# ArshvirSk/Multimodal-Rare-Disease

Hardware: NVIDIA B200
Metric: fused fwd samples/sec (224² img+128 tok) @1/2/4/8 B200; % tensor-pipe peak (higher is better)
Workload: dtype bf16

## Files before the change

multimodal-rare-disease_b200/csrc/gemm_conv.cu:

```cuda

#include "gemm_conv.h"

#include <stdio.h>
#include <stdlib.h>
#include <string.h>

#include "ptx.cuh"
#include "tma_host.h"

namespace mrd {

namespace {

bool g_use_pdl = true;

int g_debug_ring = -1;
void apply_debug_env() {
    static bool done = false;
    if (done) return;
    done = true;
    if (const char* e = getenv("MRD_DEBUG_PDL")) g_use_pdl = atoi(e) != 0;
    if (const char* e = getenv("MRD_DEBUG_RING")) g_debug_ring = atoi(e);
}

constexpr int kBlockM = 128;
constexpr int kNumThreads = 352;
constexpr int kEpiThreads = 256;
constexpr int kStageBufBytes = 128 * 128;
constexpr int kSmemLimit = 232448;
constexpr int kMaxStages = 8;
constexpr int kMaxRing = 8;
constexpr int kBarBytes = 1024;

constexpr int MODE_GENERIC = 0, MODE_STEM = 1, MODE_FLAT3 = 2;

template <int BLOCK_N, int MODE>
struct Cfg {
    static constexpr bool STEM = MODE == MODE_STEM;
    static constexpr int BLOCK_K = STEM ? 32 : 64;
    static constexpr int ROW_BYTES = BLOCK_K * 2;
    static constexpr int A_STAGE = kBlockM * ROW_BYTES;
    static constexpr int B_STAGE = BLOCK_N * ROW_BYTES;
    static constexpr int STAGE = A_STAGE + B_STAGE;
    static constexpr int FIXED = 2 * kStageBufBytes + kBarBytes + 1024;
    static constexpr int TMEM_COLS = 2 * BLOCK_N;
    static constexpr uint32_t LAYOUT = STEM ? 4u : 2u;
    static constexpr uint32_t SBO = 8 * ROW_BYTES;
};

struct TileCoord {
    int n_idx, w0, h0, n0;
};

__device__ __forceinline__ TileCoord decode_tile(const ConvGemmParams& p, int tile) {
    TileCoord t;
    int m_idx = tile / p.n_tiles_n;
    t.n_idx = tile - m_idx * p.n_tiles_n;
    int tw_i = m_idx % p.tiles_w;
    int r = m_idx / p.tiles_w;
    int th_i = r % p.tiles_h;
    int img_i = r / p.tiles_h;
    t.w0 = tw_i * p.tw + p.w_shift;
    t.h0 = th_i * p.th;
    t.n0 = img_i * p.nb;
    return t;
}

constexpr int kStemRow = 192;
constexpr int kStemRows = 37;

constexpr int kLnStripeBytes = 128 * 8 * 8 + 64;

template <int BLOCK_N, int MODE, bool SPLITK = false, bool EPI2 = false, bool LNC = false, bool PAIR = false>
__global__ void __launch_bounds__(kNumThreads, 1)
conv_gemm_kernel(const __grid_constant__ ConvGemmParams p) {
    using C = Cfg<BLOCK_N, MODE>;
    constexpr bool STEM = MODE == MODE_STEM;
    constexpr bool FLAT = MODE == MODE_FLAT3;
    constexpr bool WRES = STEM || FLAT;
    const int STAGES = p.stages;
    const int RING = p.ring;
    const int a_stage_bytes = WRES ? p.a_stage_bytes : C::A_STAGE;
    constexpr int B_STAGE = PAIR ? C::B_STAGE / 2 : C::B_STAGE;
    const int b_region = WRES ? p.b_res_bytes : STAGES * B_STAGE;

    extern __shared__ uint8_t smem_raw[];
    const uint32_t smem_base = (smem_u32(smem_raw) + 1023u) & ~1023u;
    uint8_t* smem_gen = smem_raw + (smem_base - smem_u32(smem_raw));

    const uint32_t a_smem = smem_base;
    const uint32_t b_smem = a_smem + STAGES * a_stage_bytes;
    const uint32_t st_smem = b_smem + b_region;
    const uint32_t ring_smem = st_smem + 2 * kStageBufBytes;
    const uint32_t bar_smem = ring_smem + RING * kStageBufBytes;
    uint8_t* st_gen = smem_gen + (st_smem - smem_base);
    uint8_t* ring_gen = smem_gen + (ring_smem - smem_base);
    volatile uint32_t* tmem_slot =
        reinterpret_cast<volatile uint32_t*>(smem_gen + (bar_smem - smem_base) + 320);
    const uint32_t bres_bar = bar_smem + 384u;

    auto full_bar = [&](int s) { return bar_smem + 8u * s; };
    auto empty_bar = [&](int s) { return bar_smem + 64u + 8u * s; };
    auto rfull_bar = [&](int s) { return bar_smem + 128u + 8u * s; };
    auto rempty_bar = [&](int s) { return bar_smem + 192u + 8u * s; };
    auto tfull_bar = [&](int a) { return bar_smem + 256u + 8u * a; };
    auto tempty_bar = [&](int a) { return bar_smem + 272u + 8u * a; };
    auto release_acc = [&](int a) {
        if constexpr (PAIR)
            mbar_arrive_remote(mapa_shared(tempty_bar(a), 0));
        else
            mbar_arrive(tempty_bar(a));
    };

    const int warp = threadIdx.x >> 5;
    const int lane = threadIdx.x & 31;

    if (warp == 0 && lane == 0) {
        for (int i = 0; i < 4; ++i) tma_prefetch_desc(&p.a_map[i]);
        tma_prefetch_desc(&p.b_map);
        tma_prefetch_desc(&p.c_map);
        tma_prefetch_desc(&p.r_map);
        for (int s = 0; s < kMaxStages; ++s) {
            mbar_init(full_bar(s), 1);
            mbar_init(empty_bar(s), 1);
            if constexpr (PAIR) mbar_init(bar_smem + 448u + 8u * s, 1);
            if constexpr (PAIR) mbar_init(bar_smem + 440u, 1);
            mbar_init(rfull_bar(s), 1);
            mbar_init(rempty_bar(s), 1);
        }
        for (int a = 0; a < 2; ++a) {
            mbar_init(tfull_bar(a), 1);
            mbar_init(tempty_bar(a), (PAIR ? 2 : 1) * (EPI2 ? 4 * (BLOCK_N / 64) : 8));
        }
        mbar_init(bres_bar, 1);
        fence_mbar_init();
    }
    if (warp == 1) {
        if constexpr (PAIR)
            tmem_alloc_pair<C::TMEM_COLS>(bar_smem + 320);
        else
            tmem_alloc<C::TMEM_COLS>(bar_smem + 320);
    }
    tc_fence_before();
    __syncthreads();
    tc_fence_after();
    const uint32_t tmem_base = *tmem_slot;
    if constexpr (PAIR) cluster_sync_all();

    asm volatile("griddepcontrol.wait;" ::: "memory");
    asm volatile("griddepcontrol.launch_dependents;" ::: "memory");

    constexpr int NSUB = BLOCK_N / 64;
    int num_k = p.kc_split ? p.num_k_total : p.num_taps * p.kc_per_tap;
    if constexpr (SPLITK) {
        if (p.dyn_k) {
            int live_k = (__ldg(p.dyn_k) + C::BLOCK_K - 1) / C::BLOCK_K;
            live_k = live_k < 1 ? 1 : live_k;
            num_k = live_k < num_k ? live_k : num_k;
        }
    }
    const int box_rows = p.tw * p.th * p.nb;
    const uint32_t a_box_bytes = static_cast<uint32_t>(box_rows) * C::ROW_BYTES;
    const uint32_t stage_tx = a_box_bytes + B_STAGE;
    const int bid = static_cast<int>(blockIdx.x), nblk = static_cast<int>(gridDim.x);
    int total_tiles = p.total_tiles;
    if (p.dyn_rows) {
        const int live = (__ldg(p.dyn_rows) + kBlockM - 1) / kBlockM * p.n_tiles_n;
        total_tiles = live < total_tiles ? live : total_tiles;
    }
    int ksplit = 1;
    if constexpr (SPLITK) {
        ksplit = p.ksplit > 1 ? p.ksplit : 1;
        ksplit = ksplit < num_k ? ksplit : num_k;
    }
    const int total_items = SPLITK ? total_tiles * ksplit : total_tiles;
    int my_tiles = total_items > bid ? (total_items - bid + nblk - 1) / nblk : 0;
// ... 317 lines not shown
            const float m2_p = fmaxf(ssq - sum * mean_p, 0.0f);
            float2 part[8];
            const int stripe = tile_at(it) / csize;
            char* rec = reinterpret_cast<char*>(p.ln_stats) + static_cast<long long>(stripe) * kLnStripeBytes;
            float2* srow = reinterpret_cast<float2*>(rec) + row * 8;
            __stcg(srow + t.n_idx * 2 + half, make_float2(mean_p, m2_p));
            __threadfence();
            __syncwarp();
            unsigned int* cnt = reinterpret_cast<unsigned int*>(rec + 128 * 8 * 8);
            const unsigned int want = 8u * csize;
            if (lane == 0) {
                asm volatile("red.release.gpu.global.add.u32 [%0], 1;" ::"l"(cnt) : "memory");
                unsigned int seen;
                const long long t0 = clock64();
                do {
                    asm volatile("ld.acquire.gpu.global.u32 %0, [%1];" : "=r"(seen) : "l"(cnt) : "memory");
                    if (clock64() - t0 > 4000000000LL) __trap();
                } while (seen < want);
            }
            __syncwarp();
            for (int i = 0; i < npart; ++i) part[i] = __ldcg(srow + i);
            __syncwarp();
            if (lane == 0) {
                unsigned int left;
                asm volatile("atom.acq_rel.gpu.global.add.u32 %0, [%1], 1;" : "=r"(left) : "l"(cnt + 1) : "memory");
                if (left == want - 1) {
                    cnt[1] = 0;
                    asm volatile("st.release.gpu.global.u32 [%0], %1;" ::"l"(cnt), "r"(0u) : "memory");
                }
            }
            float mean = 0.0f;
            for (int i = 0; i < npart; ++i) mean += part[i].x;
            mean *= 1.0f / static_cast<float>(npart);
            float m2 = 0.0f;
            for (int i = 0; i < npart; ++i) {
                const float d = part[i].x - mean;
                m2 += part[i].y + kPartN * d * d;
            }
            const float rstd = rsqrtf(m2 * inv_n + p.ln_eps);
            for (int sub = 0; sub < NSUB; ++sub, ++q) {
                const uint32_t buf = q & 1u;
                const int col0 = t.n_idx * BLOCK_N + sub * 64 + half * 32;
                uint32_t v[32];
                tmem_ld32(tbase + sub * 64, v);
                tmem_ld_wait();
                if (sub == NSUB - 1) {
                    tc_fence_before();
                    __syncwarp();
                    if (lane == 0) release_acc(acc);
                }
                float f[32];
#pragma unroll
                for (int j = 0; j < 32; j += 4) {
                    const float4 g4 = __ldg(reinterpret_cast<const float4*>(p.ln_g + col0 + j));
                    const float4 b4 = __ldg(reinterpret_cast<const float4*>(p.ln_b + col0 + j));
                    f[j + 0] = fmaf((__uint_as_float(v[j + 0]) - mean) * rstd, g4.x, b4.x);
                    f[j + 1] = fmaf((__uint_as_float(v[j + 1]) - mean) * rstd, g4.y, b4.y);
                    f[j + 2] = fmaf((__uint_as_float(v[j + 2]) - mean) * rstd, g4.z, b4.z);
                    f[j + 3] = fmaf((__uint_as_float(v[j + 3]) - mean) * rstd, g4.w, b4.w);
                }
                if (epi_tid == 0) tma_store_wait_read<1>();
                named_bar_sync(2, kEpiThreads);
                uint8_t* st_row = st_gen + buf * kStageBufBytes + row * 128;
#pragma unroll
                for (int c = 0; c < 4; ++c) {
                    uint4 o;
                    o.x = pack_bf16(f[c * 8 + 0], f[c * 8 + 1]);
                    o.y = pack_bf16(f[c * 8 + 2], f[c * 8 + 3]);
                    o.z = pack_bf16(f[c * 8 + 4], f[c * 8 + 5]);
                    o.w = pack_bf16(f[c * 8 + 6], f[c * 8 + 7]);
                    const int chunk = (half * 4 + c) ^ (row & 7);
                    *reinterpret_cast<uint4*>(st_row + chunk * 16) = o;
                }
                fence_proxy_async_smem();
                named_bar_sync(1, kEpiThreads);
                if (epi_tid == 0) {
                    tma_store_4d(&p.c_map, st_smem + buf * kStageBufBytes, t.n_idx * BLOCK_N + sub * 64, t.w0, t.h0,
                                 t.n0);
                    tma_store_commit();
                }
            }
        }
        if (epi_tid == 0) tma_store_wait_all<0>();
    } else if (EPI2) {
        const int grp = (warp - 2) >> 2;
        const int quarter = warp & 3;
        const int row = quarter * 32 + lane;
        const bool leader = ((warp - 2) & 3) == 0 && lane == 0;
        const int bar_a = 1 + 2 * grp, bar_b = 2 + 2 * grp;
        const int wi = row % p.tw;
        const int hi = (row / p.tw) % p.th;
        const int ni = row / (p.tw * p.th);
        const bool has_res = p.has_res != 0;
        const int nq = my_tiles * NSUB;
        uint8_t* st_row = st_gen + grp * kStageBufBytes + row * 128;
        for (int q = grp; q < nq; q += 2) {
            const int sub = q % NSUB;
            const int it = q / NSUB;
            const int acc = it & 1;
            const TileCoord t = decode_tile(p, tile_at(it));
            const int col0 = t.n_idx * BLOCK_N + sub * 64;
            mbar_wait(tfull_bar(acc), (it >> 1) & 1u);
            tc_fence_after();
            uint32_t v0[32], v1[32];
            const uint32_t taddr = tmem_base + (static_cast<uint32_t>(quarter * 32) << 16) + acc * BLOCK_N + sub * 64;
            tmem_ld32(taddr, v0);
            tmem_ld32(taddr + 32, v1);
            tmem_ld_wait();
            tc_fence_before();
            __syncwarp();
            if (lane == 0) release_acc(acc);
            float f[64];
#pragma unroll
            for (int j = 0; j < 32; j += 4) {
                float4 b0 = make_float4(0.f, 0.f, 0.f, 0.f), b1 = b0;
                if (p.bias) {
                    b0 = __ldg(reinterpret_cast<const float4*>(p.bias + col0 + j));
                    b1 = __ldg(reinterpret_cast<const float4*>(p.bias + col0 + 32 + j));
                }
                f[j + 0] = __uint_as_float(v0[j + 0]) + b0.x;
                f[j + 1] = __uint_as_float(v0[j + 1]) + b0.y;
                f[j + 2] = __uint_as_float(v0[j + 2]) + b0.z;
                f[j + 3] = __uint_as_float(v0[j + 3]) + b0.w;
                f[32 + j + 0] = __uint_as_float(v1[j + 0]) + b1.x;
                f[32 + j + 1] = __uint_as_float(v1[j + 1]) + b1.y;
                f[32 + j + 2] = __uint_as_float(v1[j + 2]) + b1.z;
                f[32 + j + 3] = __uint_as_float(v1[j + 3]) + b1.w;
            }
            if (has_res) {
                const int rslot = q % RING;
                mbar_wait(rfull_bar(rslot), static_cast<uint32_t>(q / RING) & 1u);
                const uint8_t* r_row = ring_gen + rslot * kStageBufBytes + row * 128;
#pragma unroll
                for (int c = 0; c < 8; ++c) {
                    const uint4 r4 = *reinterpret_cast<const uint4*>(r_row + ((c ^ (row & 7)) << 4));
                    const float2 r0 = unpack_bf16(r4.x), r1 = unpack_bf16(r4.y),
                                 r2 = unpack_bf16(r4.z), r3 = unpack_bf16(r4.w);
                    f[c * 8 + 0] += r0.x; f[c * 8 + 1] += r0.y;
                    f[c * 8 + 2] += r1.x; f[c * 8 + 3] += r1.y;
                    f[c * 8 + 4] += r2.x; f[c * 8 + 5] += r2.y;
                    f[c * 8 + 6] += r3.x; f[c * 8 + 7] += r3.y;
                }
            }
            if (p.act == ACT_RELU) {
#pragma unroll
                for (int j = 0; j < 64; ++j) f[j] = fmaxf(f[j], 0.0f);
            } else if (p.act == ACT_GELU) {
#pragma unroll
                for (int j = 0; j < 64; ++j) f[j] = gelu_erf_fast(f[j]);
            }
            if (p.out_f32) {
                const bool row_ok = (row < box_rows) && (t.n0 + ni < p.Nimg) && (t.h0 + hi < p.Ho) &&
                                    (t.w0 + wi < p.Wo);
                if (row_ok) {
                    const long long pix =
                        (static_cast<long long>(t.n0 + ni) * p.Ho + (t.h0 + hi)) * p.Wo + (t.w0 + wi);
                    float* f32_row = p.out_f32 + pix * p.ld_f32 + col0;
#pragma unroll
                    for (int j = 0; j < 64; j += 4)
                        *reinterpret_cast<float4*>(f32_row + j) = make_float4(f[j], f[j + 1], f[j + 2], f[j + 3]);
                }
            }
            if (leader) tma_store_wait_read<0>();
            named_bar_sync(bar_b, 128);
#pragma unroll
            for (int c = 0; c < 8; ++c) {
// ... 104 lines not shown
                const uint8_t* r_row = ring_gen + rslot * kStageBufBytes + row * 128;
#pragma unroll
                for (int c = 0; c < 4; ++c) {
                    const int chunk = (half * 4 + c) ^ (row & 7);
                    const uint4 r4 = *reinterpret_cast<const uint4*>(r_row + chunk * 16);
                    const float2 r0 = unpack_bf16(r4.x), r1 = unpack_bf16(r4.y),
                                 r2 = unpack_bf16(r4.z), r3 = unpack_bf16(r4.w);
                    f[c * 8 + 0] += r0.x; f[c * 8 + 1] += r0.y;
                    f[c * 8 + 2] += r1.x; f[c * 8 + 3] += r1.y;
                    f[c * 8 + 4] += r2.x; f[c * 8 + 5] += r2.y;
                    f[c * 8 + 6] += r3.x; f[c * 8 + 7] += r3.y;
                }
            }
            if (p.act == ACT_RELU) {
#pragma unroll
                for (int j = 0; j < 32; ++j) f[j] = fmaxf(f[j], 0.0f);
            } else if (p.act == ACT_GELU) {
#pragma unroll
                for (int j = 0; j < 32; ++j) f[j] = gelu_erf_fast(f[j]);
            }
            if (p.out_f32) {
                const bool row_ok = (row < box_rows) && (t.n0 + ni < p.Nimg) && (t.h0 + hi < p.Ho) &&
                                    (t.w0 + wi < p.Wo);
                if (row_ok) {
                    const long long pix =
                        (static_cast<long long>(t.n0 + ni) * p.Ho + (t.h0 + hi)) * p.Wo + (t.w0 + wi);
                    float* f32_row = p.out_f32 + pix * p.ld_f32 + col0;
                    if constexpr (SPLITK) {
#pragma unroll
                        for (int j = 0; j < 32; j += 4)
                            atomicAdd(reinterpret_cast<float4*>(f32_row + j),
                                      make_float4(f[j], f[j + 1], f[j + 2], f[j + 3]));
                    } else {
#pragma unroll
                        for (int j = 0; j < 32; j += 4)
                            *reinterpret_cast<float4*>(f32_row + j) =
                                make_float4(f[j], f[j + 1], f[j + 2], f[j + 3]);
                    }
                }
            }
            if (epi_tid == 0) tma_store_wait_read<1>();
            named_bar_sync(2, kEpiThreads);
            uint8_t* st_row = st_gen + buf * kStageBufBytes + row * 128;
#pragma unroll
            for (int c = 0; c < 4; ++c) {
                uint4 o;
                o.x = pack_bf16(f[c * 8 + 0], f[c * 8 + 1]);
                o.y = pack_bf16(f[c * 8 + 2], f[c * 8 + 3]);
                o.z = pack_bf16(f[c * 8 + 4], f[c * 8 + 5]);
                o.w = pack_bf16(f[c * 8 + 6], f[c * 8 + 7]);
                const int chunk = (half * 4 + c) ^ (row & 7);
                *reinterpret_cast<uint4*>(st_row + chunk * 16) = o;
            }
            fence_proxy_async_smem();
            named_bar_sync(1, kEpiThreads);
            if (has_res) {
                if (epi_tid == 0) mbar_arrive(rempty_bar(rslot));
                if (++rslot == RING) { rslot = 0; rphase ^= 1u; }
            }
            if (epi_tid == 0 && p.store_bf16) {
                if (p.c_blocked)
                    tma_store_4d(&p.c_map, st_smem + buf * kStageBufBytes, 0, t.w0, t.n_idx * NSUB + sub, 0);
                else
                    tma_store_4d(&p.c_map, st_smem + buf * kStageBufBytes, t.n_idx * BLOCK_N + sub * 64,
                                 t.w0, t.h0, t.n0);
                tma_store_commit();
            }
        }
        if (epi_tid == 0) tma_store_wait_all<0>();
    }

    tc_fence_before();
    __syncthreads();
    if constexpr (PAIR) cluster_sync_all();
    if (warp == 1) {
        tc_fence_after();
        if constexpr (PAIR)
            tmem_dealloc_pair<C::TMEM_COLS>(tmem_base);
        else
            tmem_dealloc<C::TMEM_COLS>(tmem_base);
    }
}

template <int BLOCK_N, int MODE, bool SPLITK = false, bool EPI2 = false, bool LNC = false, bool PAIR = false>
int launch_variant(const GemmLaunch* g, cudaStream_t stream) {
    using C = Cfg<BLOCK_N, MODE>;
    static bool attr_set = false;
    auto kfn = conv_gemm_kernel<BLOCK_N, MODE, SPLITK, EPI2, LNC, PAIR>;
    if (!attr_set) {
        cudaError_t e =
            cudaFuncSetAttribute(kfn, cudaFuncAttributeMaxDynamicSharedMemorySize, kSmemLimit);
        if (e != cudaSuccess) {
            set_last_error("cudaFuncSetAttribute(smem=%d): %s", kSmemLimit, cudaGetErrorString(e));
            return -static_cast<int>(e);
        }
        attr_set = true;
    }
    const int smem = MODE != MODE_GENERIC
                         ? C::FIXED + g->p.stages * g->p.a_stage_bytes + g->p.b_res_bytes
                         : C::FIXED + g->p.stages * (PAIR ? C::A_STAGE + C::B_STAGE / 2 : C::STAGE) +
                               g->p.ring * kStageBufBytes;
    cudaLaunchConfig_t cfg = {};
    cfg.gridDim = dim3(g->grid);
    cfg.blockDim = dim3(kNumThreads);
    cfg.dynamicSmemBytes = smem;
    cfg.stream = stream;
    cudaLaunchAttribute attr[2];
    attr[0].id = cudaLaunchAttributeProgrammaticStreamSerialization;
    attr[0].val.programmaticStreamSerializationAllowed = g_use_pdl ? 1 : 0;
    cfg.attrs = attr;
    cfg.numAttrs = 1;
    if (PAIR) {
        constexpr int cs = 2;
        attr[1].id = cudaLaunchAttributeClusterDimension;
        attr[1].val.clusterDim.x = cs;
        attr[1].val.clusterDim.y = 1;
        attr[1].val.clusterDim.z = 1;
        cfg.numAttrs = 2;
        static int max_clusters = 0;
        if (max_clusters == 0) {
            cfg.gridDim = dim3(cs * 16);
            int n = 0;
            cudaError_t e = cudaOccupancyMaxActiveClusters(&n, kfn, &cfg);
            if (e != cudaSuccess || n <= 0) {
                set_last_error("cudaOccupancyMaxActiveClusters(cluster of %d): %s", cs, cudaGetErrorString(e));
                return e != cudaSuccess ? -static_cast<int>(e) : -1;
            }
            max_clusters = n;
            if (getenv("MRD_DEBUG_PRINT"))
                fprintf(stderr, "[mrd] conv_gemm_kernel<%d,%d,%d,%d,%d,%d>: %d co-resident clusters of %d CTAs\n", BLOCK_N,
                        MODE, SPLITK, EPI2, LNC, PAIR, n, cs);
        }
        int clusters = g->grid / cs;
        if (clusters > max_clusters) clusters = max_clusters;
        if (clusters < 1) clusters = 1;
        cfg.gridDim = dim3(clusters * cs);
    }
    cudaError_t e = cudaLaunchKernelEx(&cfg, kfn, g->p);
    if (e == cudaSuccess) e = cudaGetLastError();
    if (e != cudaSuccess) {
        set_last_error("conv_gemm_kernel<%d,%d> launch: %s", BLOCK_N, MODE,
                       cudaGetErrorString(e));
        return -static_cast<int>(e);
    }
    return 0;
}

void pick_pipeline(ConvGemmParams* p, int block_n, bool stem, bool pair = false) {
    const int stage = stem ? (128 * 64 + 64 * 64) : (128 * 128 + (pair ? block_n / 2 : block_n) * 128);
    const int fixed = 2 * kStageBufBytes + kBarBytes + 1024;
    const int avail = kSmemLimit - fixed;
    const int num_k = p->num_taps * p->kc_per_tap;
    if (!p->has_res) {
        int s = avail / stage;
        p->stages = s > kMaxStages ? kMaxStages : s;
        if (const char* e = getenv("MRD_DEBUG_STAGES")) {
            const int v = atoi(e);
            if (v >= 2 && v < p->stages) p->stages = v;
        }
        p->ring = 0;
        return;
    }
    int s = num_k <= 2 ? 2 : 3;
    while (s > 2 && (avail - s * stage) / kStageBufBytes < 2) --s;
    int r = (avail - s * stage) / kStageBufBytes;
    if (r > kMaxRing) {
        r = kMaxRing;
        int extra = (avail - r * kStageBufBytes) / stage;
        if (extra > s) s = extra > kMaxStages ? kMaxStages : extra;
    }
    if (num_k > 6 && r > 4) {
        r = 4;
        int more = (avail - r * kStageBufBytes) / stage;
        if (more > s) s = more > kMaxStages ? kMaxStages : more;
    }
    apply_debug_env();
    if (g_debug_ring > 0 && g_debug_ring < r) r = g_debug_ring;
    p->stages = s;
    p->ring = r;
}

#define MRD_GEMM_TRY(expr)          \
    do {                            \
        int rc__ = (expr);          \
        if (rc__ != 0) return rc__; \
    } while (0)

int pick_block_n(int n, long long m_tiles, int sms) {
    if (n % 256 == 0 && m_tiles * (n / 256) >= sms) return 256;
    if (n % 128 == 0 && m_tiles * (n / 128) >= sms) return 128;
    if (n % 64 == 0 && (n % 128 != 0 || m_tiles * (n / 128) < sms)) return 64;
    if (n % 128 == 0) return 128;
    return 64;
}

int finish_plan(GemmLaunch* g, int block_n) {
    ConvGemmParams& p = g->p;
    g->block_n = block_n;
    p.n_tiles_n = p.Cout / block_n;
    const long long m_tiles = static_cast<long long>(p.tiles_w) * p.tiles_h * p.tiles_img;
    const long long total = m_tiles * p.n_tiles_n;
    if (total <= 0 || total > 0x7fffffffLL) {
        set_last_error("gemm plan: bad tile count %lld", total);
        return -1;
    }
    p.total_tiles = static_cast<int>(total);
    const int sms = gemm_num_sms();
    g->grid = p.total_tiles < sms ? p.total_tiles : sms;
    if (g->flat3 || g->stem) {
        g->grid = g->grid / p.n_tiles_n * p.n_tiles_n;
        if (g->grid < p.n_tiles_n) g->grid = p.n_tiles_n;
    } else {
        pick_pipeline(&p, block_n, false, g->pair != 0);
    }
    return 0;
}

}

void gemm_set_pdl(bool on) { g_use_pdl = on; }

int gemm_num_sms() {
    static int sms = 0;
    if (sms == 0) {
        int dev = 0;
        if (cudaGetDevice(&dev) != cudaSuccess ||
            cudaDeviceGetAttribute(&sms, cudaDevAttrMultiProcessorCount, dev) != cudaSuccess ||
            sms <= 0)
            sms = 148;
    }
    return sms;
}

namespace {
int plan_gemm_impl(GemmLaunch* g, const __nv_bfloat16* A, long long lda, int M, int K,
                   const __nv_bfloat16* W, int N, const float* bias, __nv_bfloat16* Cout, long long ldc,
                   const __nv_bfloat16* residual, long long ld_res, float* out_f32, long long ld_f32,
                   int act, int c_blocked, int force_bn);
}

int plan_gemm(GemmLaunch* g, const __nv_bfloat16* A, long long lda, int M, int K,
              const __nv_bfloat16* W, int N, const float* bias, __nv_bfloat16* Cout, long long ldc,
              const __nv_bfloat16* residual, long long ld_res, float* out_f32, long long ld_f32,
              int act, int c_blocked) {
    return plan_gemm_impl(g, A, lda, M, K, W, N, bias, Cout, ldc, residual, ld_res, out_f32, ld_f32, act, c_blocked, 0);
}

namespace {
int plan_gemm_impl(GemmLaunch* g, const __nv_bfloat16* A, long long lda, int M, int K,
                   const __nv_bfloat16* W, int N, const float* bias, __nv_bfloat16* Cout, long long ldc,
                   const __nv_bfloat16* residual, long long ld_res, float* out_f32, long long ld_f32,
                   int act, int c_blocked, int force_bn) {
    memset(g, 0, sizeof(*g));
    if (M <= 0 || K <= 0 || N <= 0 || K % 64 != 0 || N % 64 != 0 || lda % 8 != 0 ||
        (Cout && ldc % 8 != 0)) {
        set_last_error("plan_gemm: unsupported shape M=%d N=%d K=%d lda=%lld ldc=%lld", M, N, K,
                       lda, ldc);
        return -1;
    }
    ConvGemmParams& p = g->p;
    g->stem = 0;
    p.bias = bias;
    p.has_res = residual != nullptr;
    p.out_f32 = out_f32;
    p.ld_f32 = ld_f32;
    p.num_taps = 1;
    p.kc_per_tap = K / 64;
    p.taps[0] = TapDesc{0, 0, 0, 0};
    p.tw = 128; p.th = 1; p.nb = 1;
    p.tiles_w = (M + 127) / 128; p.tiles_h = 1; p.tiles_img = 1;
    p.Wo = M; p.Ho = 1; p.Nimg = 1; p.Cout = N;
    p.act = act;
    p.store_bf16 = Cout != nullptr;
    g->flops = 2.0 * M * static_cast<double>(N) * K;
    g->bytes = 2.0 * (1.0 * M * K + 1.0 * N * K + (Cout ? 1.0 * M * N : 0.0) + (residual ? 1.0 * M * N : 0.0)) +
               (out_f32 ? 4.0 * M * N : 0.0);

    const int bn = force_bn ? force_bn : pick_block_n(N, p.tiles_w, gemm_num_sms());
    g->pair = (bn == 256 && static_cast<long long>(p.tiles_w) * (N / 256) >= 2LL * gemm_num_sms()) ? 1 : 0;
    {
        uint64_t dims[4] = {(uint64_t)K, (uint64_t)M, 1, 1};
        uint64_t str[3] = {(uint64_t)lda * 2, (uint64_t)lda * 2 * M, (uint64_t)lda * 2 * M};
        uint32_t box[4] = {64, 128, 1, 1};
        int rc = encode_tensor_map(&p.a_map[0], A, 2, 4, dims, str, box, 128);
        if (rc) return rc;
        for (int i = 1; i < 4; ++i) p.a_map[i] = p.a_map[0];
    }
    {
        uint64_t dims[2] = {(uint64_t)K, (uint64_t)N};
        uint64_t str[1] = {(uint64_t)K * 2};
        uint32_t box[2] = {64, (uint32_t)(g->pair ? bn / 2 : bn)};
        int rc = encode_tensor_map(&p.b_map, W, 2, 2, dims, str, box, 128);
        if (rc) return rc;
    }
    p.c_blocked = (Cout && c_blocked) ? 1 : 0;
    if (Cout && c_blocked) {
// ... 409 lines not shown
    p.act = act;
    p.store_bf16 = 1;
    g->flops = 2.0 * N * Ho * Wo * 64.0 * 147.0;
    g->bytes = 2.0 * (1.0 * N * (H + 6) * (W + 8) * 4 + 64.0 * 7 * 32 + 1.0 * N * Ho * Wo * 64);
    if (Wo % 8 != 0 || Ho % 16 != 0) {
        set_last_error("plan_stem: output %dx%d must be a multiple of the 8 x 16 tile", Wo, Ho);
        return -1;
    }
    p.tw = 8;
    p.th = 16;
    p.nb = 1;
    p.tiles_w = Wo / 8;
    p.tiles_h = Ho / 16;
    p.tiles_img = N;
    {
        uint64_t dims[3] = {(uint64_t)Wp * 4, (uint64_t)Hp, (uint64_t)N};
        uint64_t str[2] = {(uint64_t)Wp * 8, (uint64_t)Hp * Wp * 8};
        uint32_t box[3] = {kStemRow / 2, kStemRows, 1};
        int rc = encode_tensor_map(&p.a_map[0], Xpad, 2, 3, dims, str, box, 0);
        if (rc) return rc;
        for (int i = 1; i < 4; ++i) p.a_map[i] = p.a_map[0];
    }
    {
        uint64_t dims[2] = {7 * 32, 64};
        uint64_t str[1] = {7 * 32 * 2};
        uint32_t box[2] = {32, 64};
        int rc = encode_tensor_map(&p.b_map, Wst, 2, 2, dims, str, box, 64);
        if (rc) return rc;
    }
    {
        uint64_t dims[4] = {64, (uint64_t)Wo, (uint64_t)Ho, (uint64_t)N};
        uint64_t str[3] = {64 * 2, (uint64_t)Wo * 64 * 2, (uint64_t)Ho * Wo * 64 * 2};
        uint32_t box[4] = {64, (uint32_t)p.tw, (uint32_t)p.th, 1};
        int rc = encode_tensor_map(&p.c_map, Y, 2, 4, dims, str, box, 128);
        if (rc) return rc;
        p.r_map = p.c_map;
    }
    p.a_stage_bytes = 7168;
    p.b_res_bytes = 7 * 64 * 64;
    p.ring = 0;
    p.stages = kMaxStages;
    return finish_plan(g, 64);
}

int plan_stem_pool(GemmLaunch* g, const __nv_bfloat16* Xpad, int N, int H, int W,
                   const __nv_bfloat16* Wst, const float* bias, __nv_bfloat16* P) {
    int rc = plan_stem(g, Xpad, N, H, W, Wst, bias, P, ACT_RELU);
    if (rc) return rc;
    g->p.pool_out = P;
    g->p.pool_h = H / 4;
    g->p.pool_w = W / 4;
    g->p.store_bf16 = 0;
    g->bytes = 2.0 * (1.0 * N * (H + 6) * (W + 8) * 4 + 64.0 * 7 * 32 + 1.0 * N * (H / 4) * (W / 4) * 64);
    return 0;
}

int launch_gemm(const GemmLaunch* g, cudaStream_t stream) {
    apply_debug_env();
    if (g->stem) {
        if (g->p.pool_out) return launch_variant<64, MODE_STEM, false, true>(g, stream);
        return launch_variant<64, MODE_STEM>(g, stream);
    }
    if (g->lnc)
        return g->pair ? launch_variant<256, MODE_GENERIC, false, false, true, true>(g, stream)
                       : launch_variant<256, MODE_GENERIC, false, false, true>(g, stream);
    if (g->flat3 && g->pair)
        return g->block_n == 128 ? launch_variant<128, MODE_FLAT3, false, true, false, true>(g, stream)
                                 : launch_variant<64, MODE_FLAT3, false, true, false, true>(g, stream);
    if (g->flat3) {
        switch (g->block_n) {
            case 64: return launch_variant<64, MODE_FLAT3, false, true>(g, stream);
            case 128: return launch_variant<128, MODE_FLAT3, false, true>(g, stream);
        }
        set_last_error("launch_gemm: bad flat3 block_n %d", g->block_n);
        return -1;
    }
    if (g->p.f32_accum) {
        switch (g->block_n) {
            case 64: return launch_variant<64, MODE_GENERIC, true>(g, stream);
            case 128: return launch_variant<128, MODE_GENERIC, true>(g, stream);
            case 256: return launch_variant<256, MODE_GENERIC, true>(g, stream);
        }
    }
    const bool chain_bound = g->p.act == ACT_GELU || g->p.num_taps * g->p.kc_per_tap <= 6 ||
                             (g->p.kc_split && g->p.num_k_total <= 6);
    const bool epi2 = chain_bound && !(g->p.kc_split && g->p.num_k_total > 6);
    if (g->pair && g->block_n == 256) {
        if (epi2) return launch_variant<256, MODE_GENERIC, false, true, false, true>(g, stream);
        return launch_variant<256, MODE_GENERIC, false, false, false, true>(g, stream);
    }
    if (epi2) {
        switch (g->block_n) {
            case 64: return launch_variant<64, MODE_GENERIC, false, true>(g, stream);
            case 128: return launch_variant<128, MODE_GENERIC, false, true>(g, stream);
            case 256: return launch_variant<256, MODE_GENERIC, false, true>(g, stream);
        }
    }
    switch (g->block_n) {
        case 64: return launch_variant<64, MODE_GENERIC>(g, stream);
        case 128: return launch_variant<128, MODE_GENERIC>(g, stream);
        case 256: return launch_variant<256, MODE_GENERIC>(g, stream);
    }
    set_last_error("launch_gemm: bad block_n %d", g->block_n);
    return -1;
}

}
```

multimodal-rare-disease_b200/csrc/ptx.cuh:

```cuda
#pragma once

#include <cuda.h>
#include <cuda_runtime.h>
#include <cuda_bf16.h>
#include <stdint.h>

namespace mrd {

__device__ __forceinline__ uint32_t smem_u32(const void* p) {
    return static_cast<uint32_t>(__cvta_generic_to_shared(p));
}

__device__ __forceinline__ int lane_id() { return threadIdx.x & 31; }

__device__ __forceinline__ void mbar_init(uint32_t bar, uint32_t count) {
    asm volatile("mbarrier.init.shared::cta.b64 [%0], %1;" ::"r"(bar), "r"(count) : "memory");
}

__device__ __forceinline__ void fence_mbar_init() {
    asm volatile("fence.mbarrier_init.release.cluster;" ::: "memory");
}

__device__ __forceinline__ void mbar_expect_tx(uint32_t bar, uint32_t bytes) {
    asm volatile("mbarrier.arrive.expect_tx.shared::cta.b64 _, [%0], %1;" ::"r"(bar), "r"(bytes)
// ... 138 lines not shown
    asm volatile("cp.async.bulk.commit_group;" ::: "memory");
}
template <int N>
__device__ __forceinline__ void tma_store_wait_read() {
    asm volatile("cp.async.bulk.wait_group.read %0;" ::"n"(N) : "memory");
}
template <int N>
__device__ __forceinline__ void tma_store_wait_all() {
    asm volatile("cp.async.bulk.wait_group %0;" ::"n"(N) : "memory");
}

template <int NCOLS>
__device__ __forceinline__ void tmem_alloc(uint32_t smem_result_addr) {
    asm volatile("tcgen05.alloc.cta_group::1.sync.aligned.shared::cta.b32 [%0], %1;" ::"r"(
                     smem_result_addr),
                 "n"(NCOLS)
                 : "memory");
    asm volatile("tcgen05.relinquish_alloc_permit.cta_group::1.sync.aligned;" ::: "memory");
}
template <int NCOLS>
__device__ __forceinline__ void tmem_dealloc(uint32_t taddr) {
    asm volatile("tcgen05.dealloc.cta_group::1.sync.aligned.b32 %0, %1;" ::"r"(taddr), "n"(NCOLS)
                 : "memory");
}

template <int NCOLS>
__device__ __forceinline__ void tmem_alloc_pair(uint32_t smem_result_addr) {
    asm volatile("tcgen05.alloc.cta_group::2.sync.aligned.shared::cta.b32 [%0], %1;" ::"r"(smem_result_addr),
                 "n"(NCOLS)
                 : "memory");
    asm volatile("tcgen05.relinquish_alloc_permit.cta_group::2.sync.aligned;" ::: "memory");
}
template <int NCOLS>
__device__ __forceinline__ void tmem_dealloc_pair(uint32_t taddr) {
    asm volatile("tcgen05.dealloc.cta_group::2.sync.aligned.b32 %0, %1;" ::"r"(taddr), "n"(NCOLS) : "memory");
}
__device__ __forceinline__ void umma_bf16_pair(uint32_t tmem_d, uint64_t desc_a, uint64_t desc_b, uint32_t idesc,
                                               uint32_t accumulate) {
    asm volatile(
        "{\n\t.reg .pred p;\n\t"
        "setp.ne.b32 p, %4, 0;\n\t"
        "tcgen05.mma.cta_group::2.kind::f16 [%0], %1, %2, %3, p;\n\t}" ::"r"(tmem_d),
        "l"(desc_a), "l"(desc_b), "r"(idesc), "r"(accumulate)
        : "memory");
}
__device__ __forceinline__ void umma_commit_pair(uint32_t bar, uint16_t cta_mask) {
    asm volatile(
        "tcgen05.commit.cta_group::2.mbarrier::arrive::one.shared::cluster.multicast::cluster.b64 [%0], %1;" ::"r"(bar),
        "h"(cta_mask)
        : "memory");
}

__device__ __forceinline__ void umma_bf16(uint32_t tmem_d, uint64_t desc_a, uint64_t desc_b,
                                          uint32_t idesc, uint32_t accumulate) {
    asm volatile(
        "{\n\t.reg .pred p;\n\t"
        "setp.ne.b32 p, %4, 0;\n\t"
        "tcgen05.mma.cta_group::1.kind::f16 [%0], %1, %2, %3, p;\n\t}" ::"r"(tmem_d),
        "l"(desc_a), "l"(desc_b), "r"(idesc), "r"(accumulate)
        : "memory");
}

__device__ __forceinline__ void umma_commit(uint32_t bar) {
    asm volatile("tcgen05.commit.cta_group::1.mbarrier::arrive::one.shared::cluster.b64 [%0];" ::
                     "r"(bar)
                 : "memory");
}

__device__ __forceinline__ void tmem_ld32(uint32_t taddr, uint32_t (&v)[32]) {
    asm volatile(
        "tcgen05.ld.sync.aligned.32x32b.x32.b32 "
        "{%0, %1, %2, %3, %4, %5, %6, %7, %8, %9, %10, %11, %12, %13, %14, %15, "
        "%16, %17, %18, %19, %20, %21, %22, %23, %24, %25, %26, %27, %28, %29, %30, %31}, [%32];"
        : "=r"(v[0]), "=r"(v[1]), "=r"(v[2]), "=r"(v[3]), "=r"(v[4]), "=r"(v[5]), "=r"(v[6]),
          "=r"(v[7]), "=r"(v[8]), "=r"(v[9]), "=r"(v[10]), "=r"(v[11]), "=r"(v[12]), "=r"(v[13]),
          "=r"(v[14]), "=r"(v[15]), "=r"(v[16]), "=r"(v[17]), "=r"(v[18]), "=r"(v[19]),
          "=r"(v[20]), "=r"(v[21]), "=r"(v[22]), "=r"(v[23]), "=r"(v[24]), "=r"(v[25]),
          "=r"(v[26]), "=r"(v[27]), "=r"(v[28]), "=r"(v[29]), "=r"(v[30]), "=r"(v[31])
        : "r"(taddr)
        : "memory");
}
__device__ __forceinline__ void tmem_ld_wait() {
    asm volatile("tcgen05.wait::ld.sync.aligned;" ::: "memory");
}

__device__ __forceinline__ void tmem_st32(uint32_t taddr, const uint32_t (&v)[32]) {
    asm volatile(
        "tcgen05.st.sync.aligned.32x32b.x32.b32 [%0], "
        "{%1, %2, %3, %4, %5, %6, %7, %8, %9, %10, %11, %12, %13, %14, %15, %16, "
        "%17, %18, %19, %20, %21, %22, %23, %24, %25, %26, %27, %28, %29, %30, %31, %32};" ::"r"(taddr),
        "r"(v[0]), "r"(v[1]), "r"(v[2]), "r"(v[3]), "r"(v[4]), "r"(v[5]), "r"(v[6]), "r"(v[7]), "r"(v[8]), "r"(v[9]),
        "r"(v[10]), "r"(v[11]), "r"(v[12]), "r"(v[13]), "r"(v[14]), "r"(v[15]), "r"(v[16]), "r"(v[17]), "r"(v[18]),
        "r"(v[19]), "r"(v[20]), "r"(v[21]), "r"(v[22]), "r"(v[23]), "r"(v[24]), "r"(v[25]), "r"(v[26]), "r"(v[27]),
        "r"(v[28]), "r"(v[29]), "r"(v[30]), "r"(v[31])
        : "memory");
}
__device__ __forceinline__ void tmem_st_wait() {
    asm volatile("tcgen05.wait::st.sync.aligned;" ::: "memory");
}

__device__ __forceinline__ uint32_t cluster_ctarank() {
    uint32_t r;
    asm volatile("mov.u32 %0, %%cluster_ctarank;" : "=r"(r));
    return r;
}
__device__ __forceinline__ void cluster_sync_all() {
    asm volatile("barrier.cluster.arrive.release.aligned;\n\tbarrier.cluster.wait.acquire.aligned;" ::: "memory");
}
__device__ __forceinline__ uint32_t mapa_shared(uint32_t addr, uint32_t rank) {
    uint32_t r;
    asm volatile("mapa.shared::cluster.u32 %0, %1, %2;" : "=r"(r) : "r"(addr), "r"(rank));
    return r;
}
__device__ __forceinline__ void tma_load_2d_multicast(const void* map, uint32_t bar, uint32_t dst, int c0, int c1,
                                                      uint16_t cta_mask) {
    asm volatile(
        "cp.async.bulk.tensor.2d.shared::cluster.global.mbarrier::complete_tx::bytes.multicast::cluster"
        " [%0], [%1, {%3, %4}], [%2], %5;" ::"r"(dst),
        "l"(reinterpret_cast<uint64_t>(map)), "r"(bar), "r"(c0), "r"(c1), "h"(cta_mask)
        : "memory");
}
__device__ __forceinline__ void umma_commit_multicast(uint32_t bar, uint16_t cta_mask) {
    asm volatile(
        "tcgen05.commit.cta_group::1.mbarrier::arrive::one.shared::cluster.multicast::cluster.b64 [%0], %1;" ::"r"(bar),
        "h"(cta_mask)
        : "memory");
}
__device__ __forceinline__ void mbar_arrive_remote(uint32_t cluster_bar) {
    asm volatile("mbarrier.arrive.shared::cluster.b64 _, [%0];" ::"r"(cluster_bar) : "memory");
}

__device__ __forceinline__ uint64_t make_smem_desc(uint32_t saddr, uint32_t lbo_bytes,
                                                   uint32_t sbo_bytes, uint32_t layout) {
    uint64_t d = 0;
    d |= static_cast<uint64_t>((saddr >> 4) & 0x3FFF);
    d |= static_cast<uint64_t>((lbo_bytes >> 4) & 0x3FFF) << 16;
    d |= static_cast<uint64_t>((sbo_bytes >> 4) & 0x3FFF) << 32;
    d |= 1ull << 46;
    d |= static_cast<uint64_t>(layout & 7) << 61;
    return d;
}

__host__ __device__ constexpr uint32_t make_idesc_bf16(int M, int N, int a_mn, int b_mn) {
    return (1u << 4) | (1u << 7) | (1u << 10) | (static_cast<uint32_t>(a_mn) << 15) |
           (static_cast<uint32_t>(b_mn) << 16) | (static_cast<uint32_t>(N >> 3) << 17) |
           (static_cast<uint32_t>(M >> 4) << 24);
}

__device__ __forceinline__ uint32_t pack_bf16(float lo, float hi) {
    __nv_bfloat162 t = __floats2bfloat162_rn(lo, hi);
    return *reinterpret_cast<uint32_t*>(&t);
}
__device__ __forceinline__ float2 unpack_bf16(uint32_t u) {
    __nv_bfloat162 t = *reinterpret_cast<__nv_bfloat162*>(&u);
    return __bfloat1622float2(t);
}
__device__ __forceinline__ float gelu_erf(float x) {
    return 0.5f * x * (1.0f + erff(x * 0.70710678118654752f));
}
__device__ __forceinline__ float gelu_erf_fast(float x) {
    float t, e;
    const float ax = fabsf(x);
    const float w = ax * 0.84932180028801904f;
    asm("rcp.approx.ftz.f32 %0, %1;" : "=f"(t) : "f"(fmaf(0.27273748f, w, 1.0f)));
    asm("ex2.approx.ftz.f32 %0, %1;" : "=f"(e) : "f"(w * -w));
    float poly = fmaf(0.5f * 1.061405429f, t, 0.5f * -1.453152027f);
// ... 9 lines not shown
```

Before: 37470.

## Add dedicated software-pipelined GELU epilogue for conv GEMM

Adds a GELU-specialised epilogue path that double-buffers TMEM loads: it issues the load for the next half or subtile while doing bias, residual and GELU math on the current one, and releases the accumulator earlier. Bias values are staged in a small extra shared-memory region, and a register-tied tmem_ld_wait keeps the compiler from moving uses of the loaded registers ahead of the wait. GELU layers previously went through the generic EPI2 path. The intent is to hide the TMEM load latency and the GELU math cost behind each other. The extra shared memory reduces pipeline stage capacity slightly, and the more complex barrier ordering carries some correctness risk.

```diff
diff --git a/multimodal-rare-disease_b200/csrc/gemm_conv.cu b/multimodal-rare-disease_b200/csrc/gemm_conv.cu
--- a/multimodal-rare-disease_b200/csrc/gemm_conv.cu
+++ b/multimodal-rare-disease_b200/csrc/gemm_conv.cu
@@ -31,6 +31,7 @@
 constexpr int kMaxStages = 8;
 constexpr int kMaxRing = 8;
 constexpr int kBarBytes = 1024;
+constexpr int kGeluExtraBytes = 2 * 128 * 4;
 
 constexpr int MODE_GENERIC = 0, MODE_STEM = 1, MODE_FLAT3 = 2;
 
@@ -71,7 +72,8 @@
 
 constexpr int kLnStripeBytes = 128 * 8 * 8 + 64;
 
-template <int BLOCK_N, int MODE, bool SPLITK = false, bool EPI2 = false, bool LNC = false, bool PAIR = false>
+template <int BLOCK_N, int MODE, bool SPLITK = false, bool EPI2 = false, bool LNC = false, bool PAIR = false,
+          bool GELU = false>
 __global__ void __launch_bounds__(kNumThreads, 1)
 conv_gemm_kernel(const __grid_constant__ ConvGemmParams p) {
     using C = Cfg<BLOCK_N, MODE>;
@@ -91,7 +93,7 @@
     const uint32_t a_smem = smem_base;
     const uint32_t b_smem = a_smem + STAGES * a_stage_bytes;
     const uint32_t st_smem = b_smem + b_region;
-    const uint32_t ring_smem = st_smem + 2 * kStageBufBytes;
+    const uint32_t ring_smem = st_smem + 2 * kStageBufBytes + (GELU ? kGeluExtraBytes : 0);
     const uint32_t bar_smem = ring_smem + RING * kStageBufBytes;
     uint8_t* st_gen = smem_gen + (st_smem - smem_base);
     uint8_t* ring_gen = smem_gen + (ring_smem - smem_base);
@@ -575,6 +577,136 @@
             }
         }
         if (epi_tid == 0) tma_store_wait_all<0>();
+    } else if constexpr (GELU) {
+        const int grp = (warp - 2) >> 2;
+        const int quarter = warp & 3;
+        const int row = quarter * 32 + lane;
+        const int gt = threadIdx.x - 64 - grp * 128;
+        const bool leader = gt == 0;
+        const int bar_a = 1 + 2 * grp, bar_b = 2 + 2 * grp;
+        const int wi = row % p.tw;
+        const int hi = (row / p.tw) % p.th;
+        const int ni = row / (p.tw * p.th);
+        const bool has_res = p.has_res != 0;
+        const int nq = my_tiles * NSUB;
+        constexpr int GSUB = NSUB > 1 ? NSUB / 2 : 1;
+        float* bias_s = reinterpret_cast<float*>(st_gen + 2 * kStageBufBytes) + grp * 128;
+        auto bias_of = [&](int it) -> float {
+            if (gt >= GSUB * 64 || !p.bias) return 0.0f;
+            const int sub = NSUB > 1 ? grp + 2 * (gt >> 6) : 0;
+            return __ldg(p.bias + decode_tile(p, tile_at(it)).n_idx * BLOCK_N + sub * 64 + (gt & 63));
+        };
+        auto tmem_half = [&](int q, int h) -> uint32_t {
+            return tmem_base + (static_cast<uint32_t>(quarter * 32) << 16) + ((q / NSUB) & 1) * BLOCK_N +
+                   (q % NSUB) * 64 + h * 32;
+        };
+        auto half_math = [&](const uint32_t (&v)[32], const float* bsm, const uint8_t* r_row, float* f32_row, int h,
+                             uint32_t* o) {
+            float f[32];
+#pragma unroll
+            for (int j = 0; j < 32; j += 4) {
+                const float4 b4 = *reinterpret_cast<const float4*>(bsm + j);
+                f[j + 0] = __fadd_rn(__uint_as_float(v[j + 0]), b4.x);
+                f[j + 1] = __fadd_rn(__uint_as_float(v[j + 1]), b4.y);
+                f[j + 2] = __fadd_rn(__uint_as_float(v[j + 2]), b4.z);
+                f[j + 3] = __fadd_rn(__uint_as_float(v[j + 3]), b4.w);
+            }
+            if (r_row) {
+#pragma unroll
+                for (int c = 0; c < 4; ++c) {
+                    const uint4 r4 = *reinterpret_cast<const uint4*>(r_row + (((h * 4 + c) ^ (row & 7)) << 4));
+                    const float2 r0 = unpack_bf16(r4.x), r1 = unpack_bf16(r4.y),
+                                 r2 = unpack_bf16(r4.z), r3 = unpack_bf16(r4.w);
+                    f[c * 8 + 0] = __fadd_rn(f[c * 8 + 0], r0.x); f[c * 8 + 1] = __fadd_rn(f[c * 8 + 1], r0.y);
+                    f[c * 8 + 2] = __fadd_rn(f[c * 8 + 2], r1.x); f[c * 8 + 3] = __fadd_rn(f[c * 8 + 3], r1.y);
+                    f[c * 8 + 4] = __fadd_rn(f[c * 8 + 4], r2.x); f[c * 8 + 5] = __fadd_rn(f[c * 8 + 5], r2.y);
+                    f[c * 8 + 6] = __fadd_rn(f[c * 8 + 6], r3.x); f[c * 8 + 7] = __fadd_rn(f[c * 8 + 7], r3.y);
+                }
+            }
+#pragma unroll
+            for (int j = 0; j < 32; ++j) f[j] = gelu_erf_fast(f[j]);
+            if (f32_row) {
+#pragma unroll
+                for (int j = 0; j < 32; j += 4)
+                    *reinterpret_cast<float4*>(f32_row + h * 32 + j) = make_float4(f[j], f[j + 1], f[j + 2], f[j + 3]);
+            }
+#pragma unroll
+            for (int c = 0; c < 4; ++c) {
+                o[c * 4 + 0] = pack_bf16(f[c * 8 + 0], f[c * 8 + 1]);
+                o[c * 4 + 1] = pack_bf16(f[c * 8 + 2], f[c * 8 + 3]);
+                o[c * 4 + 2] = pack_bf16(f[c * 8 + 4], f[c * 8 + 5]);
+                o[c * 4 + 3] = pack_bf16(f[c * 8 + 6], f[c * 8 + 7]);
+            }
+        };
+        uint32_t v0[32], v1[32];
+        if (grp < nq) {
+            const int it0 = grp / NSUB;
+            if (gt < GSUB * 64) bias_s[gt] = bias_of(it0);
+            mbar_wait(tfull_bar(it0 & 1), (it0 >> 1) & 1u);
+            tc_fence_after();
+            tmem_ld32(tmem_half(grp, 0), v0);
+            named_bar_sync(bar_a, 128);
+            tmem_ld_wait(v0);
+        }
+        for (int q = grp; q < nq; q += 2) {
+            const int sub = q % NSUB;
+            const int it = q / NSUB;
+            const int acc = it & 1;
+            const int j = NSUB > 1 ? sub >> 1 : 0;
+            const bool more = q + 2 < nq;
+            const bool next_same_tile = more && (q + 2) / NSUB == it;
+            const bool new_bias = more && j == GSUB - 1;
+            const float bias_next = new_bias ? bias_of((q + 2) / NSUB) : 0.0f;
+            const TileCoord t = decode_tile(p, tile_at(it));
+            const int col0 = t.n_idx * BLOCK_N + sub * 64;
+            tmem_ld32(tmem_half(q, 1), v1);
+            const uint8_t* r_row = nullptr;
+            if (has_res) {
+                const int rslot = q % RING;
+                mbar_wait(rfull_bar(rslot), static_cast<uint32_t>(q / RING) & 1u);
+                r_row = ring_gen + rslot * kStageBufBytes + row * 128;
+            }
+            float* f32_row = nullptr;
+            if (p.out_f32 && row < box_rows && t.n0 + ni < p.Nimg && t.h0 + hi < p.Ho && t.w0 + wi < p.Wo)
+                f32_row = p.out_f32 +
+                          ((static_cast<long long>(t.n0 + ni) * p.Ho + (t.h0 + hi)) * p.Wo + (t.w0 + wi)) * p.ld_f32 +
+                          col0;
+            uint32_t o[32];
+            half_math(v0, bias_s + j * 64, r_row, f32_row, 0, o);
+            tmem_ld_wait(v1);
+            tc_fence_before();
+            __syncwarp();
+            if (lane == 0) release_acc(acc);
+            if (next_same_tile) tmem_ld32(tmem_half(q + 2, 0), v0);
+            half_math(v1, bias_s + j * 64 + 32, r_row, f32_row, 1, o + 16);
+            const uint32_t buf = static_cast<uint32_t>(grp);
+            if (leader) tma_store_wait_read<0>();
+            named_bar_sync(bar_b, 128);
+            uint8_t* st_row = st_gen + buf * kStageBufBytes + row * 128;
+#pragma unroll
+            for (int c = 0; c < 8; ++c)
+                *reinterpret_cast<uint4*>(st_row + ((c ^ (row & 7)) << 4)) =
+                    make_uint4(o[c * 4 + 0], o[c * 4 + 1], o[c * 4 + 2], o[c * 4 + 3]);
+            if (new_bias && gt < GSUB * 64) bias_s[gt] = bias_next;
+            fence_proxy_async_smem();
+            named_bar_sync(bar_a, 128);
+            if (leader && has_res) mbar_arrive(rempty_bar(q % RING));
+            if (leader && p.store_bf16) {
+                if (p.c_blocked)
+                    tma_store_4d(&p.c_map, st_smem + buf * kStageBufBytes, 0, t.w0, t.n_idx * NSUB + sub, 0);
+                else
+                    tma_store_4d(&p.c_map, st_smem + buf * kStageBufBytes, col0, t.w0, t.h0, t.n0);
+                tma_store_commit();
+            }
+            if (more && !next_same_tile) {
+                const int it2 = (q + 2) / NSUB;
+                mbar_wait(tfull_bar(it2 & 1), (it2 >> 1) & 1u);
+                tc_fence_after();
+                tmem_ld32(tmem_half(q + 2, 0), v0);
+            }
+            if (more) tmem_ld_wait(v0);
+        }
+        if (leader) tma_store_wait_all<0>();
     } else if (EPI2) {
         const int grp = (warp - 2) >> 2;
         const int quarter = warp & 3;
@@ -845,11 +977,12 @@
     }
 }
 
-template <int BLOCK_N, int MODE, bool SPLITK = false, bool EPI2 = false, bool LNC = false, bool PAIR = false>
+template <int BLOCK_N, int MODE, bool SPLITK = false, bool EPI2 = false, bool LNC = false, bool PAIR = false,
+          bool GELU = false>
 int launch_variant(const GemmLaunch* g, cudaStream_t stream) {
     using C = Cfg<BLOCK_N, MODE>;
     static bool attr_set = false;
-    auto kfn = conv_gemm_kernel<BLOCK_N, MODE, SPLITK, EPI2, LNC, PAIR>;
+    auto kfn = conv_gemm_kernel<BLOCK_N, MODE, SPLITK, EPI2, LNC, PAIR, GELU>;
     if (!attr_set) {
         cudaError_t e =
             cudaFuncSetAttribute(kfn, cudaFuncAttributeMaxDynamicSharedMemorySize, kSmemLimit);
@@ -861,8 +994,8 @@
     }
     const int smem = MODE != MODE_GENERIC
                          ? C::FIXED + g->p.stages * g->p.a_stage_bytes + g->p.b_res_bytes
-                         : C::FIXED + g->p.stages * (PAIR ? C::A_STAGE + C::B_STAGE / 2 : C::STAGE) +
-                               g->p.ring * kStageBufBytes;
+                         : C::FIXED + (GELU ? kGeluExtraBytes : 0) +
+                               g->p.stages * (PAIR ? C::A_STAGE + C::B_STAGE / 2 : C::STAGE) + g->p.ring * kStageBufBytes;
     cudaLaunchConfig_t cfg = {};
     cfg.gridDim = dim3(g->grid);
     cfg.blockDim = dim3(kNumThreads);
@@ -891,8 +1024,8 @@
             }
             max_clusters = n;
             if (getenv("MRD_DEBUG_PRINT"))
-                fprintf(stderr, "[mrd] conv_gemm_kernel<%d,%d,%d,%d,%d,%d>: %d co-resident clusters of %d CTAs\n", BLOCK_N,
-                        MODE, SPLITK, EPI2, LNC, PAIR, n, cs);
+                fprintf(stderr, "[mrd] conv_gemm_kernel<%d,%d,%d,%d,%d,%d,%d>: %d co-resident clusters of %d CTAs\n",
+                        BLOCK_N, MODE, SPLITK, EPI2, LNC, PAIR, GELU, n, cs);
         }
         int clusters = g->grid / cs;
         if (clusters > max_clusters) clusters = max_clusters;
@@ -909,9 +1042,9 @@
     return 0;
 }
 
-void pick_pipeline(ConvGemmParams* p, int block_n, bool stem, bool pair = false) {
+void pick_pipeline(ConvGemmParams* p, int block_n, bool stem, bool pair = false, bool gelu = false) {
     const int stage = stem ? (128 * 64 + 64 * 64) : (128 * 128 + (pair ? block_n / 2 : block_n) * 128);
-    const int fixed = 2 * kStageBufBytes + kBarBytes + 1024;
+    const int fixed = 2 * kStageBufBytes + kBarBytes + 1024 + (gelu ? kGeluExtraBytes : 0);
     const int avail = kSmemLimit - fixed;
     const int num_k = p->num_taps * p->kc_per_tap;
     if (!p->has_res) {
@@ -974,7 +1107,7 @@
         g->grid = g->grid / p.n_tiles_n * p.n_tiles_n;
         if (g->grid < p.n_tiles_n) g->grid = p.n_tiles_n;
     } else {
-        pick_pipeline(&p, block_n, false, g->pair != 0);
+        pick_pipeline(&p, block_n, false, g->pair != 0, p.act == ACT_GELU);
     }
     return 0;
 }
@@ -1550,8 +1683,18 @@
             case 256: return launch_variant<256, MODE_GENERIC, true>(g, stream);
         }
     }
-    const bool chain_bound = g->p.act == ACT_GELU || g->p.num_taps * g->p.kc_per_tap <= 6 ||
-                             (g->p.kc_split && g->p.num_k_total <= 6);
+    if (g->p.act == ACT_GELU) {
+        if (g->pair && g->block_n == 256)
+            return launch_variant<256, MODE_GENERIC, false, true, false, true, true>(g, stream);
+        switch (g->block_n) {
+            case 64: return launch_variant<64, MODE_GENERIC, false, true, false, false, true>(g, stream);
+            case 128: return launch_variant<128, MODE_GENERIC, false, true, false, false, true>(g, stream);
+            case 256: return launch_variant<256, MODE_GENERIC, false, true, false, false, true>(g, stream);
+        }
+        set_last_error("launch_gemm: bad block_n %d", g->block_n);
+        return -1;
+    }
+    const bool chain_bound = g->p.num_taps * g->p.kc_per_tap <= 6 || (g->p.kc_split && g->p.num_k_total <= 6);
     const bool epi2 = chain_bound && !(g->p.kc_split && g->p.num_k_total > 6);
     if (g->pair && g->block_n == 256) {
         if (epi2) return launch_variant<256, MODE_GENERIC, false, true, false, true>(g, stream);
diff --git a/multimodal-rare-disease_b200/csrc/ptx.cuh b/multimodal-rare-disease_b200/csrc/ptx.cuh
--- a/multimodal-rare-disease_b200/csrc/ptx.cuh
+++ b/multimodal-rare-disease_b200/csrc/ptx.cuh
@@ -244,6 +244,16 @@
 }
 __device__ __forceinline__ void tmem_ld_wait() {
     asm volatile("tcgen05.wait::ld.sync.aligned;" ::: "memory");
+}
+__device__ __forceinline__ void tmem_ld_wait(uint32_t (&v)[32]) {
+    asm volatile(
+        "tcgen05.wait::ld.sync.aligned;"
+        : "+r"(v[0]), "+r"(v[1]), "+r"(v[2]), "+r"(v[3]), "+r"(v[4]), "+r"(v[5]), "+r"(v[6]), "+r"(v[7]),
+          "+r"(v[8]), "+r"(v[9]), "+r"(v[10]), "+r"(v[11]), "+r"(v[12]), "+r"(v[13]), "+r"(v[14]), "+r"(v[15]),
+          "+r"(v[16]), "+r"(v[17]), "+r"(v[18]), "+r"(v[19]), "+r"(v[20]), "+r"(v[21]), "+r"(v[22]), "+r"(v[23]),
+          "+r"(v[24]), "+r"(v[25]), "+r"(v[26]), "+r"(v[27]), "+r"(v[28]), "+r"(v[29]), "+r"(v[30]), "+r"(v[31])
+        :
+        : "memory");
 }
 
 __device__ __forceinline__ void tmem_st32(uint32_t taddr, const uint32_t (&v)[32]) {
```

After: 37570, median of 6. Within noise of the previous version (+0.3%).
